# google/ffn

Hardware: AMD Instinct MI355X
Metric: FoV-steps/sec (flood-filling inference loop, 250^3 volume) (higher is better)
Workload: dtype f32 (fp16 hi + scaled-residual split products on the fp16 MFMA, f32 accumulate)

## Files before the change

ffn_amd/_lib.py:

```python

from __future__ import annotations

import ctypes
import os
import subprocess
import threading

_HERE = os.path.dirname(os.path.abspath(__file__))
CSRC = os.path.join(_HERE, 'csrc')
LIB_PATH = os.environ.get('FFN_AMD_LIB') or os.path.join(CSRC, 'libffn_hip.so')
HEADER = os.path.join(os.path.dirname(_HERE), 'include', 'ffn_hip.h')
HEADERS = [HEADER,
           os.path.join(os.path.dirname(_HERE), 'include', 'ffn_hip_debug.h'),
           os.path.join(os.path.dirname(_HERE), 'include', 'ffn_labels.h'),
           os.path.join(os.path.dirname(_HERE), 'include', 'ffn_seeds.h'),
           os.path.join(os.path.dirname(_HERE), 'include', 'ffn_decision.h'),
           os.path.join(os.path.dirname(_HERE), 'include', 'ffn_analysis.h'),
           os.path.join(os.path.dirname(_HERE), 'include', 'ffn_partitions.h'),
           os.path.join(os.path.dirname(_HERE), 'include', 'ffn_coordinates.h'),
           os.path.join(os.path.dirname(_HERE), 'include', 'ffn_evaluation.h'),
           os.path.join(os.path.dirname(_HERE), 'include', 'ffn_gradients.h'),
           os.path.join(os.path.dirname(_HERE), 'include', 'ffn_optimizer.h')]
SOURCES = ['ffn_hip.hip', 'ffn_canvas.hip', 'ffn_options.hip', 'ffn_labels.hip',
           'ffn_seeds.hip', 'ffn_decision.hip', 'ffn_analysis.hip',
# ... 81 lines not shown
              ('seed_got_too_weak', ctypes.c_int32),
              ('budget_exhausted', ctypes.c_int32),
              ('active', ctypes.c_int32),
              ('start_logit_known', ctypes.c_int32),
              ('start_logit', ctypes.c_float),
              ('min_pos', ctypes.c_int32 * 3),
              ('max_pos', ctypes.c_int32 * 3)]


class CommitCounts(ctypes.Structure):
  _fields_ = [('raw_segmented_voxels', ctypes.c_int64),
              ('actual_segmented_voxels', ctypes.c_int64),
              ('num_overlapped_ids', ctypes.c_int32)]


class TurnRequest(ctypes.Structure):
  _fields_ = [('do_commit', ctypes.c_int32),
              ('lo', ctypes.c_int32 * 3), ('hi', ctypes.c_int32 * 3),
              ('segment_threshold', ctypes.c_float),
              ('min_segment_size', ctypes.c_int64),
              ('segment_id', ctypes.c_int32),
              ('max_existing_id', ctypes.c_int32),
              ('mark_mode', ctypes.c_int32),
              ('mark_pos', ctypes.c_int32 * 3),
              ('num_candidates', ctypes.c_int32),
              ('min_boundary_dist', ctypes.c_int32 * 3),
              ('do_init', ctypes.c_int32),
              ('init_value', ctypes.c_float)]


class TurnResult(ctypes.Structure):
  _fields_ = [('counts', CommitCounts), ('committed', ctypes.c_int32),
              ('chosen', ctypes.c_int32)]


class PairDesc(ctypes.Structure):
  _fields_ = [('probs', ctypes.c_void_p), ('seg', ctypes.c_void_p),
              ('id_a', ctypes.c_uint64), ('id_b', ctypes.c_uint64),
              ('box_zyx', ctypes.c_int32 * 3), ('off_zyx', ctypes.c_int32 * 3),
              ('shape_zyx', ctypes.c_int32 * 3), ('reserved', ctypes.c_int32)]


class EvaluationSectionPlan(ctypes.Structure):
  _fields_ = [('margin_yx', ctypes.c_int32 * 2), ('kind', ctypes.c_int32),
              ('z0', ctypes.c_int32), ('dy', ctypes.c_int32),
              ('dx', ctypes.c_int32), ('blank_value', ctypes.c_float),
              ('blur_sigma', ctypes.c_float)]


class EvaluationSection(ctypes.Structure):
  _fields_ = [('blank_mask', ctypes.c_uint8), ('blur_mask', ctypes.c_uint8),
              ('gray', ctypes.c_uint8), ('reserved', ctypes.c_uint8),
              ('blank_yx', ctypes.c_int32 * 2), ('blur_yx', ctypes.c_int32 * 2),
              ('contrast', ctypes.c_float), ('brightness', ctypes.c_float),
              ('gamma', ctypes.c_float)]


class EvaluationGeometry(ctypes.Structure):
  _fields_ = [('input_seed_zyx', ctypes.c_int32 * 3),
              ('input_image_zyx', ctypes.c_int32 * 3),
              ('pred_mask_zyx', ctypes.c_int32 * 3),
              ('deltas_zyx', ctypes.c_int32 * 3),
              ('canvas_zyx', ctypes.c_int32 * 3),
              ('image_patch_zyx', ctypes.c_int32 * 3),
              ('label_patch_zyx', ctypes.c_int32 * 3),
              ('eval_zyx', ctypes.c_int32 * 3),
# ... 20 lines not shown
    'ffn_engine_set_weights': (_I, [_P, _P, ctypes.c_size_t]),
    'ffn_engine_set_pred_size': (_I, [_P, _I3]),
    'ffn_engine_set_option': (_I, [_P, ctypes.c_char_p, _I]),
    'ffn_engine_get_option': (_I, [_P, ctypes.c_char_p,
                                   ctypes.POINTER(ctypes.c_int)]),
    'ffn_engine_set_profiling': (_I, [_P, _I]),
    'ffn_engine_get_profile': (_I, [_P, ctypes.POINTER(ctypes.c_double),
                                    ctypes.POINTER(ctypes.c_int64), _I]),
    'ffn_engine_get_profile_samples': (_I, [_P, _P, _I, _P]),
    'ffn_engine_synchronize': (_I, [_P]),
    'ffn_engine_debug_clocks': (_I, [_P, _P]),
    'ffn_engine_debug_workgroups': (_I, [_P, _P, _I]),
    'ffn_engine_debug_flow_trace': (_I, [_P, _P, _I]),
    'ffn_predict': (_I, [_P, _I, _P, _P, _P]),
    'ffn_predict_device': (_I, [_P, _I, _P, _P, _P]),
    'ffn_forward_resident': (_I, [_P, _I, _I]),
    'ffn_canvas_create': (_I, [_P, _P, _I3, ctypes.POINTER(_P)]),
    'ffn_canvas_create_u8': (_I, [_P, _P, _I3, ctypes.c_float, ctypes.c_float,
                                  ctypes.POINTER(_P)]),
    'ffn_canvas_destroy': (None, [_P]),
    'ffn_canvas_init_seed': (_I, [_P, _I3, ctypes.c_float]),
    'ffn_canvas_step': (_I, [_P, _I, ctypes.POINTER(_P),
                             ctypes.POINTER(StepRequest),
                             ctypes.POINTER(StepParams),
                             ctypes.POINTER(StepResult)]),
    'ffn_canvas_step_submit': (_I, [_P, _I, ctypes.POINTER(_P),
                                    ctypes.POINTER(StepRequest),
                                    ctypes.POINTER(StepParams),
                                    ctypes.POINTER(ctypes.c_uint32)]),
    'ffn_canvas_step_wait': (_I, [_P, ctypes.c_uint32,
                                  ctypes.POINTER(StepResult)]),
    'ffn_canvas_segment_at': (_I, [_P, _I3, ctypes.POINTER(SegmentParams), _I,
                                   ctypes.POINTER(SegmentResult)]),
    'ffn_canvas_segment_many': (_I, [_P, _I, _P, _P, _P, _P, _P, _P]),
    'ffn_canvas_segment_many_carry': (_I, [_P, _I, _P, _P, _P, _P, _P, _P,
                                           ctypes.c_int32]),
    'ffn_canvas_segment_history': (_I, [_P, ctypes.c_size_t, ctypes.c_size_t,
                                        _P, _P,
                                        ctypes.POINTER(ctypes.c_size_t)]),
    'ffn_canvas_read_points': (_I, [_P, _I, _P, _P, _P]),
    'ffn_canvas_write_seg_points': (_I, [_P, _I, _P, _P]),
    'ffn_canvas_any_segmented': (_I, [_P, _I3, _I3,
                                      ctypes.POINTER(ctypes.c_int32)]),
    'ffn_canvas_commit_count': (_I, [_P, _I3, _I3, ctypes.c_float,
                                     ctypes.c_int32,
                                     ctypes.POINTER(CommitCounts),
                                     ctypes.c_int32, _P, _P]),
    'ffn_canvas_commit_assign': (_I, [_P, _I3, _I3, ctypes.c_float,
                                      ctypes.c_int32]),
    'ffn_canvas_segment_turn': (_I, [_P, _P, _P, _P, ctypes.c_int32, _P, _P, _P, _P,
                                     _P]),
    'ffn_canvas_set_restrictor': (_I, [_P, _P, _P, _P, _I3, _I3, _I3,
                                       ctypes.c_int32]),
    'ffn_canvas_read_restriction': (_I, [_P, _I3, _I3, _P]),
    'ffn_canvas_take_restricted_skips': (_I, [_P,
                                              ctypes.POINTER(ctypes.c_int64)]),
    'ffn_canvas_read_seed': (_I, [_P, _I3, _I3, _P]),
    'ffn_canvas_read_segmentation': (_I, [_P, _I3, _I3, _P]),
    'ffn_canvas_write_seed': (_I, [_P, _I3, _I3, _P]),
    'ffn_canvas_write_segmentation': (_I, [_P, _I3, _I3, _P]),
    'ffn_labels_create': (_I, [_I, ctypes.POINTER(_P)]),
    'ffn_labels_destroy': (None, [_P]),
    'ffn_labels_pair_counts': (_I, [_P, _P, _P, _I, ctypes.c_size_t,
                                    ctypes.c_size_t, _P, _P, _P, _P,
                                    ctypes.POINTER(ctypes.c_size_t)]),
    'ffn_labels_apply_pair_labels': (_I, [_P, ctypes.c_size_t, _P, _P, _P]),
# ... 238 lines not shown
```

ffn_amd/csrc/ffn_engine.h:

```cpp
#ifndef FFN_ENGINE_H_
#define FFN_ENGINE_H_

#include <hip/hip_runtime.h>

#include <algorithm>
#include <chrono>
#include <cstdarg>
#include <cstdio>
#include <mutex>
#include <vector>

#include "ffn_internal.h"
#include "ffn_types.h"
#include "ffn_stack_plan.h"
#include "ffn_host_loop.h"

using namespace ffn;

__attribute__((format(printf, 2, 3))) inline int fail(int code, const char* fmt, ...) {
  char buf[512];
  va_list ap;
  va_start(ap, fmt);
  vsnprintf(buf, sizeof(buf), fmt, ap);
  va_end(ap);
// ... 143 lines not shown
  unsigned long long* h_turn_dev = nullptr;
  size_t turn_ncap = 0, turn_hcap = 0, turn_ocap = 0;
  bool turn_hist_clean = false;
  unsigned turn_seq = 0;

  int prof_mode = 0;
  std::vector<hipEvent_t> events;
  int events_used = 0;
  hipEvent_t ahead_ev[2] = {nullptr, nullptr};
  bool ahead_ev_pending = false;
  double conv_ms = 0.0;
  int64_t conv_launches = 0;
  std::vector<ffn_canvas*> canvases;
  int prof_every = 1;
  long stack_calls = 0;
  bool prof_now = false;
  int ablate = 0;
  std::vector<int> chain_launches_pending;
  std::vector<float> prof_samples;
};

struct ffn_canvas {
  ffn_engine* engine = nullptr;
  float* image = nullptr;
  uint8_t* image_u8 = nullptr;
  float* image_lut = nullptr;
  float* seed = nullptr;
  int32_t* seg = nullptr;
  int cz = 0, cy = 0, cx = 0;
  size_t nvox = 0;
  int dirty_lo[3] = {0, 0, 0};
  int dirty_hi[3] = {0, 0, 0};
  ffn_host::SegmentState loop;
  hipEvent_t ev_util = nullptr;
  bool util_pending = false;
  bool paste_after_flag = false;
  int hint_n = 0;
  int hint_pos[kSpecMax][3] = {};
  bool hint_from_loop = false;
  unsigned long long* restrict_planes = nullptr;
  size_t restrict_plane_words = 0;
  int restrict_row_words = 0;
  std::vector<uint64_t> restrict_host;

  void mark_dirty(const int lo[3], const int hi[3]) {
    const int dims[3] = {cz, cy, cx};
    const bool empty = dirty_lo[0] >= dirty_hi[0];
    for (int k = 0; k < 3; ++k) {
      const int l = std::max(lo[k], 0), h = std::min(hi[k], dims[k]);
      dirty_lo[k] = empty ? l : std::min(dirty_lo[k], l);
      dirty_hi[k] = empty ? h : std::max(dirty_hi[k], h);
    }
  }
};

inline long long steady_ns() {
  return std::chrono::duration_cast<std::chrono::nanoseconds>(
             std::chrono::steady_clock::now().time_since_epoch()).count();
}
inline unsigned next_tag(unsigned t) { return t + 1 ? t + 1 : 1; }
inline void drop_spec(ffn_engine* e) {
  if (e->spec.valid && !e->ahead_valid) e->range_tag = next_tag(e->range_tag);
  if (e->ahead_valid) e->stat_ahead_wasted += 1;
  e->spec.valid = false;
  e->ahead_valid = false;
}
// ... 132 lines not shown
```

ffn_amd/csrc/ffn_hip.hip:

```cpp

#include <hip/hip_runtime.h>
#include <hip/hip_ext.h>

#include <algorithm>
#include <cmath>
#include <cstdarg>
#include <cstdio>
#include <cstdlib>
#include <cstring>
#include <map>
#include <mutex>
#include <string>
#include <vector>

#include "ffn_engine.h"
#include "ffn_kernels.h"
#include "ffn_step_kernels.h"
#include "ffn_conv_exact.h"
#include "ffn_conv_split.h"
#include "ffn_conv_resident.h"
#include "ffn_conv_half.h"

namespace {
thread_local std::string g_error;
// ... 1640 lines not shown
    drop_spec(e);
  }
  rc = ffn_canvas_step_submit(e, n, canvases, requests, params, &ticket);
  if (rc) return rc;
  return step_wait_impl(e, ticket, results, nullptr);
}

namespace {
int check_segment_params(const ffn_canvas* c, const ffn_segment_params& p, int resume, int k) {
  if (p.prefetch < 0 || p.prefetch > FFN_MAX_CANDIDATES)
    return fail(FFN_ERR_ARG, "prefetch must be 0..%d", FFN_MAX_CANDIDATES);
  if (p.shape_zyx[0] != c->cz || p.shape_zyx[1] != c->cy || p.shape_zyx[2] != c->cx)
    return k < 0 ? fail(FFN_ERR_ARG, "shape_zyx does not match the canvas")
                 : fail(FFN_ERR_ARG, "shape_zyx does not match canvas %d", k);
  for (int a = 0; a < 3; ++a)
    if (p.deltas_zyx[a] < 0 || p.margin_zyx[a] < 0)
      return fail(FFN_ERR_ARG, "negative deltas / margin");
  if (resume && !c->loop.active)
    return k < 0 ? fail(FFN_ERR_STATE, "no segment to resume")
                 : fail(FFN_ERR_STATE, "canvas %d: no segment to resume", k);
  return FFN_OK;
}

struct HipLoopDevice {
  ffn_canvas* c;
  int step(const ffn_step_request& req, const ffn_step_params& params,
           ffn_step_result* res) {
    ffn_canvas* one = c;
    return ffn_canvas_step(c->engine, 1, &one, &req, &params, res);
  }
  int read_point(const int32_t pos[3], float* seed, int32_t* seg) {
    return ffn_canvas_read_points(c, 1, pos, seed, seg);
  }
  void hint_next(int n, const int32_t (*pos)[3]) {
    EngineLock lock_(c->engine);
    c->hint_from_loop = true;
    c->hint_n = n < kSpecMax ? n : kSpecMax;
    for (int j = 0; j < c->hint_n; ++j)
      for (int a = 0; a < 3; ++a) c->hint_pos[j][a] = pos[j][a];
  }
};
}

namespace {
int resolve_many_carry_locked(ffn_engine* e) {
  if (!e->many_carry.active) return FFN_OK;
  HipLoopDevice dev{e->many_canvases.empty() ? nullptr : e->many_canvases[0]};
  auto wait = [&](ffn_step_result* res) {
    return step_wait_impl(e, e->many_ticket, res, nullptr);
  };
  const int rc = ffn_host::resolve_carry(&e->many_carry, dev, wait);
  e->many_canvases.clear();
  return rc;
}
}

}

int resolve_many_carry(ffn_engine* e, const ffn_canvas* only) {
  std::lock_guard<std::mutex> guard(e->many_mu);
  if (only && std::find(e->many_canvases.begin(), e->many_canvases.end(), only) ==
                  e->many_canvases.end())
    return FFN_OK;
  return resolve_many_carry_locked(e);
}

extern "C" {

int ffn_canvas_segment_at(ffn_canvas* c, const int32_t start[3],
                          const ffn_segment_params* p, int resume,
                          ffn_segment_result* out) {
  if (!c || !start || !p || !out) return fail(FFN_ERR_ARG, "null argument");
  if (!c->engine) return fail(FFN_ERR_STATE, "canvas outlived its engine");
  if (int rc = resolve_many_carry(c->engine, c)) return rc;
  if (int rc = check_segment_params(c, *p, resume, -1)) return rc;
  HipLoopDevice dev{c};
  ffn_host::SegmentLoop<HipLoopDevice> loop(dev, c->loop, *p);
  return loop.run(start, resume, out);
}

int ffn_canvas_segment_many(ffn_engine* e, int n, ffn_canvas* const* canvases,
                            const int32_t (*starts)[3],
                            const ffn_segment_params* params, const int32_t* resume,
                            ffn_segment_result* results, int32_t* finished) {
  return ffn_canvas_segment_many_carry(e, n, canvases, starts, params, resume, results,
                                       finished, 0);
}

int ffn_canvas_segment_many_carry(ffn_engine* e, int n, ffn_canvas* const* canvases,
                                  const int32_t (*starts)[3],
                                  const ffn_segment_params* params,
                                  const int32_t* resume, ffn_segment_result* results,
                                  int32_t* finished, int32_t carry) {
  if (!e || !canvases || !starts || !params || !resume || !results || !finished)
    return fail(FFN_ERR_ARG, "null argument");
  if (n < 1 || n > e->max_batch)
    return fail(FFN_ERR_ARG, "batch %d outside [1, %d]", n, e->max_batch);
  std::vector<HipLoopDevice> devs(n);
  std::vector<ffn_host::SegmentState*> states(n);
  for (int k = 0; k < n; ++k) {
    ffn_canvas* c = canvases[k];
    if (!c) return fail(FFN_ERR_ARG, "null canvas");
    if (c->engine != e) return fail(FFN_ERR_ARG, "canvas %d is not of this engine", k);
    for (int k2 = 0; k2 < k; ++k2)
      if (canvases[k2] == c) return fail(FFN_ERR_ARG, "canvas appears twice");
    const ffn_segment_params& p = params[k];
    if (int rc = check_segment_params(c, p, resume[k], k)) return rc;
    if (std::memcmp(&p.step, &params[0].step, sizeof(ffn_step_params)) != 0)
      return fail(FFN_ERR_ARG, "canvas %d: step parameters differ from canvas 0's", k);
    devs[k].c = c;
    states[k] = &c->loop;
// ... 38 lines not shown
```

ffn_amd/csrc/ffn_host_loop.h:

```cpp
#pragma once

#include <cstdlib>
#include <algorithm>
#include <cstdint>
#include <cstring>
#include <deque>
#include <unordered_map>
#include <unordered_set>
#include <vector>

#include "../../include/ffn_hip.h"

namespace ffn_host {

struct Coord {
  int32_t z, y, x;
  bool operator==(const Coord& o) const { return z == o.z && y == o.y && x == o.x; }
};

struct CoordHash {
  size_t operator()(const Coord& c) const {
    uint64_t h = (uint64_t)(uint32_t)c.z * 0x9E3779B97F4A7C15ull;
    h ^= (uint64_t)(uint32_t)c.y * 0xC2B2AE3D27D4EB4Full + (h << 6) + (h >> 2);
    h ^= (uint64_t)(uint32_t)c.x * 0x165667B19E3779F9ull + (h << 6) + (h >> 2);
    return (size_t)h;
  }
};

inline int32_t floordiv(int32_t a, int32_t b) {
  int32_t q = a / b;
  if ((a % b != 0) && (a < 0)) --q;
  return q;
}

struct SegmentState {
  struct Entry {
// ... 352 lines not shown
        m.rel[axis] = off;
        m.rel[o0] = fi - d_[o0];
        m.rel[o1] = fj - d_[o1];
        m.seg = res.face_seg[k];
        moves[nm++] = m;
      }
    }
    std::sort(moves, moves + nm, [](const Move& a, const Move& b) {
      if (a.score != b.score) return a.score > b.score;
      for (int i = 0; i < 3; ++i)
        if (a.rel[i] != b.rel[i]) return a.rel[i] > b.rel[i];
      return a.seg > b.seg;
    });
    for (int i = 0; i < nm; ++i) {
      if (i > 0 && moves[i].score == moves[i - 1].score &&
          moves[i].rel[0] == moves[i - 1].rel[0] &&
          moves[i].rel[1] == moves[i - 1].rel[1] &&
          moves[i].rel[2] == moves[i - 1].rel[2])
        continue;
      const Coord c{moves[i].rel[0] + pos.z, moves[i].rel[1] + pos.y,
                    moves[i].rel[2] + pos.x};
      push(moves[i].score, c);
      st_.cache.emplace(c, std::make_pair(moves[i].score, moves[i].seg));
    }
  }

  Dev& dev_;
  SegmentState& st_;
  const ffn_segment_params& p_;
  int32_t d_[3], dh_[3], dm_[3];
  int64_t steps_ = 0;
};

template <class Dev, class Wait>
int resolve_carry(ManyCarry* carry, Dev& any_dev, Wait&& wait) {
  if (!carry || !carry->active) return FFN_OK;
  std::vector<ffn_step_result> res(carry->items.size());
  const int rc = wait(res.data());
  carry->active = false;
  if (rc == FFN_OK) {
    for (size_t b = 0; b < carry->items.size(); ++b) {
      ManyCarry::Item& it = carry->items[b];
      SegmentLoop<Dev> loop(any_dev, *it.st, it.params);
      loop.consume(it.pd, res[b]);
      it.st->many_steps += 1;
    }
  }
  carry->items.clear();
  return rc;
}

template <class Dev, class BatchStep, class Submit, class Wait>
int segment_many(int n, Dev* devs, SegmentState* const* states,
                 const int32_t (*starts)[3], const ffn_segment_params* params,
                 const int32_t* resume, ffn_segment_result* out, int32_t* finished,
                 BatchStep&& batch_step, ManyCarry* carry, Submit&& submit,
                 Wait&& wait) {
  typedef SegmentLoop<Dev> Loop;
  for (int k = 1; k < n; ++k)
    if (std::memcmp(&params[k].step, &params[0].step, sizeof(ffn_step_params)) != 0)
      return FFN_ERR_ARG;
  const int rc_carry = resolve_carry(carry, devs[0], wait);
  std::vector<Loop> loops;
  loops.reserve(n);
  std::vector<char> running(n, 1);
  std::vector<typename Loop::Pending> pend(n);
// ... 76 lines not shown
```

ffn_amd/engine.py:

```python

from __future__ import annotations

import atexit
import ctypes
import threading
from typing import Sequence
import weakref

import numpy as np

from . import _lib
from ._lib import (CommitCounts, StepParams, StepRequest, StepResult, check, i3)


def _f32(a):
  return np.ascontiguousarray(a, dtype=np.float32)


_LIVE_ENGINES = weakref.WeakSet()


@atexit.register
def _close_all_engines():
  for eng in list(_LIVE_ENGINES):
# ... 16 lines not shown


def segment_many_with_retry(once, n, sarr, parr, rarr, before, fallback):
  res = (_lib.SegmentResult * n)()
  fin = (ctypes.c_int32 * n)()
  keys = list(range(n))
  sa, pa, ra, cur_res, cur_fin = sarr, parr, rarr, res, fin
  for attempt in range(MAX_VOID_REPEATS + 1):
    rc = once(keys, sa, pa, ra, cur_res, cur_fin)
    if cur_res is not res:
      for j, k in enumerate(keys):
        ctypes.pointer(res[k])[0] = cur_res[j]
        fin[k] = cur_fin[j]
    if rc not in _lib.ERR_VOIDED or attempt == MAX_VOID_REPEATS:
      return rc, res, fin
    fallback(rc)
    keys = [k for k in keys if not fin[k]]
    if not keys:
      return 0, res, fin
    m = len(keys)
    sa = (ctypes.c_int32 * 3 * m)()
    pa = (_lib.SegmentParams * m)()
    ra = (ctypes.c_int32 * m)(*([1] * m))
    cur_res = (_lib.SegmentResult * m)()
    cur_fin = (ctypes.c_int32 * m)()
    for j, k in enumerate(keys):
      for a in range(3):
        sa[j][a] = sarr[k][a]
      ctypes.pointer(pa[j])[0] = parr[k]
      if parr[k].max_steps > 0:
        spent = int(res[k].num_steps) - before[k]
        pa[j].max_steps = max(parr[k].max_steps - spent, 1)
  return rc, res, fin


class HipEngine:

  def __init__(self, fov_zyx, deltas_zyx, depth: int, features: int = 32,
               max_batch: int = 1, device_id: int = 0):
    self._lib = _lib.load()
    self._h = ctypes.c_void_p()
    self.fov_zyx = tuple(int(v) for v in fov_zyx)
    self.deltas_zyx = tuple(int(v) for v in deltas_zyx)
    self.depth = int(depth)
    self.features = int(features)
    self.max_batch = int(max_batch)
    self.device_id = int(device_id)
    check(self._lib.ffn_engine_create(self.device_id, i3(self.fov_zyx),
                                      i3(self.deltas_zyx), self.depth,
                                      self.features, self.max_batch,
                                      ctypes.byref(self._h)))
    self._canvas_arr = (ctypes.c_void_p * self.max_batch)()
    self._req_arr = (StepRequest * self.max_batch)()
    self._res_arr = (StepResult * self.max_batch)()
    self._slot_canvas_arr = [(ctypes.c_void_p * self.max_batch)()
                             for _ in range(2)]
    self._slot_req_arr = [(StepRequest * self.max_batch)() for _ in range(2)]
    self._slot_res_arr = [(StepResult * self.max_batch)() for _ in range(2)]
    self._submit_slot = 0
    self._ticket_slot = {}
    self._step_lock = threading.RLock()
    self.range_fallbacks = 0
    self.flow_fallbacks = 0
    self.variant_is_explicit = False
    self._default_variant = self.get_option('conv_variant')
    self.pred_zyx = self.fov_zyx
# ... 267 lines not shown
  def init_seed(self, pos, value: float):
    check(self._lib.ffn_canvas_init_seed(self._h, i3(pos), float(value)))

  def read_point(self, pos):
    self._pt[0], self._pt[1], self._pt[2] = int(pos[0]), int(pos[1]), int(pos[2])
    check(self._lib.ffn_canvas_read_points(
        self._h, 1, ctypes.addressof(self._pt), ctypes.addressof(self._pt_seed),
        ctypes.addressof(self._pt_seg)))
    return self._pt_seed.value, self._pt_seg.value

  def segment_at(self, start_pos, params: '_lib.SegmentParams',
                 resume: bool = False) -> '_lib.SegmentResult':
    res = _lib.SegmentResult()
    rc = self._lib.ffn_canvas_segment_at(self._h, i3(start_pos),
                                         ctypes.byref(params), int(resume),
                                         ctypes.byref(res))
    budget = params.max_steps
    summed = ('num_steps', 'skip_threshold', 'skip_invalid_pos', 'gate_rejects')
    before = dict.fromkeys(summed, 0)
    for _ in range(MAX_VOID_REPEATS):
      if rc not in _lib.ERR_VOIDED:
        break
      self.engine.voided(rc)
      for name in summed:
        before[name] += getattr(res, name)
      if budget > 0:
        params.max_steps = max(budget - before['num_steps'], 1)
      rc = self._lib.ffn_canvas_segment_at(self._h, i3(start_pos),
                                           ctypes.byref(params), 1,
                                           ctypes.byref(res))
    params.max_steps = budget
    for name in summed:
      setattr(res, name, getattr(res, name) + before[name])
    check(rc)
    return res

  def segment_history(self):
    total = ctypes.c_size_t(0)
    check(self._lib.ffn_canvas_segment_history(self._h, 0, 0, None, None,
                                               ctypes.byref(total)))
    n = total.value
    pos = np.empty((n, 3), np.int32)
    deleted = np.empty(n, np.uint32)
    if n:
      check(self._lib.ffn_canvas_segment_history(
          self._h, 0, n, pos.ctypes.data, deleted.ctypes.data, None))
    return pos, deleted

  def read_points(self, pos: np.ndarray):
    pos = np.ascontiguousarray(pos, dtype=np.int32).reshape(-1, 3)
    seed = np.empty(len(pos), np.float32)
    seg = np.empty(len(pos), np.int32)
    if len(pos):
      check(self._lib.ffn_canvas_read_points(self._h, len(pos), pos.ctypes.data,
                                             seed.ctypes.data, seg.ctypes.data))
    return seed, seg

  def write_seg_points(self, pos: np.ndarray, values: np.ndarray):
    pos = np.ascontiguousarray(pos, dtype=np.int32).reshape(-1, 3)
    values = np.ascontiguousarray(values, dtype=np.int32).ravel()
    assert len(pos) == len(values)
    if len(pos):
      check(self._lib.ffn_canvas_write_seg_points(
          self._h, len(pos), pos.ctypes.data, values.ctypes.data))

  def any_segmented(self, lo, hi) -> bool:
# ... 124 lines not shown
```

ffn_amd/inference/inference.py:

```python

from __future__ import annotations

import collections
import inspect
import ctypes

import logging
import os
import struct
import sys
import threading
import weakref
import time

import numpy as np
from scipy.special import expit
from scipy.special import logit

from .. import _lib
from .. import engine as hip_engine
from ..training import model as ffn_model
from . import executor
from . import movement
from . import seed as seed_lib
# ... 676 lines not shown
    else:
      image = np.ascontiguousarray(self.image, dtype=np.float32)
    self._handle = self._exec_client.create_canvas(image)
    self.seed = _DeviceArray(self, 'seed')
    self.segmentation = _DeviceArray(self, 'seg')
    if self.keep_probability_maps:
      self.seg_prob = storage.NumpyArray(shape=self.shape, dtype=np.uint8)
    else:
      self.seg_prob = None

  def _call(self, fn, *args, **kwargs):
    return self._exec_client.canvas_call(fn, *args, **kwargs)

  def close(self):
    if self._handle is not None:
      self._call(self._handle.close)
      self._handle = None

  def __del__(self):
    try:
      self.close()
    except Exception:
      pass
    super().__del__()

  def _invalidate_cache(self):
    self._cache = {}
    self._cached_start = None
    self._turn_rec = None

  TURN_CANDIDATES = int(os.environ.get('FFN_AMD_TURN_CANDIDATES', '128'))

  def _turn_ok(self) -> bool:
    ok = self.__dict__.get('_turn_static')
    if ok is None:
      ok = (hasattr(self._handle, 'segment_turn') and
            not self.keep_probability_maps and self._restrictor_ok())
      self._turn_static = ok
    return (ok and not self._checkpoint_due() and self.TURN_CANDIDATES > 0 and
            getattr(self.is_valid_pos, '__func__', None)
            is DeviceCanvas.is_valid_pos)

  def _policy_list(self):
    policy = self.__dict__.get('seed_policy')
    if getattr(type(policy), '__next__', None) is not seed_lib.BaseSeedPolicy.__next__:
      return None, None
    return getattr(policy, 'coords', None), getattr(policy, 'idx', None)

  def _is_current_seed(self, pos) -> bool:
    coords, idx = self._policy_list()
    return (coords is not None and idx is not None and
            1 <= idx <= len(coords) and
            tuple(int(v) for v in coords[idx - 1]) == pos)

  def _upcoming_seeds(self, first=None):
    coords, idx = self._policy_list()
    if coords is None or idx is None:
      return [] if first is None else [first]
    if first is not None:
      if not (1 <= idx <= len(coords) and
              tuple(int(v) for v in coords[idx - 1]) == first):
        return [first]
      idx -= 1
    out, listed = [], set()
    for c in np.asarray(coords[idx:idx + self.TURN_CANDIDATES]).tolist():
      c = (int(c[0]), int(c[1]), int(c[2]))
      if not self._in_bounds(c) or c in listed:
        break
      listed.add(c)
      out.append(c)
    return out

# ... 137 lines not shown
    t_done = time.time()
    self.t_last_predict = t_done
    hot[2] += t_done - t_call
    pred = self._finish_step(res)
    hot[0] += 1
    hot[1] += time.time() - t_start
    return pred

  def update_at(self, pos):
    return self._drive(self._update_at_gen(pos))

  def segment_at(self, start_pos, dynamic_image=None, vis_update_every=10,
                 vis_fixed_z=False, partial_segment_iters=0):
    del dynamic_image, vis_update_every, vis_fixed_z
    return self._drive(self._segment_at_gen(start_pos, partial_segment_iters))

  NATIVE_LOOP = os.environ.get('FFN_AMD_NATIVE_LOOP', '1') != '0'

  def _native_loop_ok(self) -> bool:
    ok = self.__dict__.get('_native_ok')
    if ok is None:
      cls = type(self)
      ok = (cls.NATIVE_LOOP and
            hasattr(self._handle, 'segment_at') and
            getattr(self._exec_client, 'in_thread', False) and
            type(self.movement_policy) is movement.FaceMaxMovementPolicy and
            self._restrictor_ok() and
            cls._segment_at_gen is DeviceCanvas._segment_at_gen)
      self._native_ok = ok
    return (ok and
            getattr(self.update_at, '__func__', None) is DeviceCanvas.update_at
            and getattr(self.is_valid_pos, '__func__', None)
            is DeviceCanvas.is_valid_pos)

  def _segment_params(self):
    sp = self.__dict__.get('_seg_params')
    if sp is None:
      sp = _lib.SegmentParams()
      policy = self.movement_policy
      sp.score_threshold = float(policy.score_threshold)
      for a in range(3):
        sp.deltas_zyx[a] = int(policy.deltas[a])
        sp.margin_zyx[a] = int(self._margin_t[a])
        sp.shape_zyx[a] = int(self.shape[a])
      sp.prefetch = self.PREFETCH
      sp.keep_history = 1 if self._keep_history else 0
      self._seg_params = sp
    sp.step = self._step_params
    return sp

  def _native_prelude(self, start_pos, resume=False):
    sp = self._segment_params()
    if not resume:
      if self.reset_seed_per_segment:
        self.init_seed(start_pos)
      self.reset_state(start_pos, reset_extents=self.reset_seed_per_segment)
      if self.movement_policy or self._min_pos is None:
        return None
      for a in range(3):
        sp.init_min_pos[a] = int(self._min_pos[a])
        sp.init_max_pos[a] = int(self._max_pos[a])
      cs = self._cached_start
      sp.initial_start_logit = (cs[1] if cs is not None and cs[0] == start_pos
                                else float('nan'))
    return sp

# ... 189 lines not shown
      while sid in self.origins:
        sid += 1
      out = self._turn(([int(v) for v in sel_lo], [int(v) for v in sel_hi], thr,
                        int(self.options.min_segment_size), sid, max_existing),
                       (pos, 2))
      raw, actual, ids, counts, committed = out[:5]
      if not committed:
        return raw, actual, ids, counts, None
      got = self.get_next_segment_id()
      assert got == sid, (got, sid)
      return raw, actual, ids, counts, sid
    raw, actual, ids, counts = self._call(self._handle.commit_count, sel_lo,
                                          sel_hi, thr, max_existing)
    if actual < self.options.min_segment_size:
      return raw, actual, ids, counts, None
    sid = self.get_next_segment_id()
    if self.keep_probability_maps:
      sel = tuple(slice(l, h) for l, h in zip(sel_lo, sel_hi))
      seed = self._call(self._handle.read_seed, sel_lo, sel_hi)
      seg = self._call(self._handle.read_segmentation, sel_lo, sel_hi)
      mask = (seed >= thr) & (seg <= 0)
      self.seg_prob[sel][mask] = storage.quantize_probability(
          expit(seed[mask]))
    self._invalidate_cache()
    self._call(self._handle.commit_assign, sel_lo, sel_hi, thr, sid)
    return raw, actual, ids, counts, sid

  def _set_segmentation(self, seg):
    self.segmentation[...] = np.asarray(seg, np.int32)

  def _set_seed(self, seed):
    self.seed[...] = np.asarray(seed, np.float32)
    self._turn_armed = False


class NativeSegment:

  __slots__ = ('start_pos', 'params', 'started')

  def __init__(self, start_pos, params):
    self.start_pos = start_pos
    self.params = params
    self.started = False


class MultiCanvasDriver:

  def __init__(self, engine, batch_size=None, overlap=True,
               max_steps_per_canvas=None, native=None, groups=1, carry=None):
    self.engine = engine
    hip_engine.pin_batched_arithmetic(engine)
    self.batch_size = batch_size or engine.max_batch
    self.overlap = overlap
    if native is None:
      native = os.environ.get('FFN_AMD_NATIVE_MANY', '1') != '0'
    self.native = bool(native) and hasattr(engine, 'segment_many')
    self.groups = max(1, int(groups)) if self.native else 1
    if carry is None:
      carry = os.environ.get('FFN_AMD_MANY_CARRY', '1') != '0'
    self.carry = bool(carry)
    self.max_steps_per_canvas = max_steps_per_canvas
    self.calls = 0
    self.steps = 0
    self.library_seconds = 0.0
    self.segments_ended = 0

# ... 249 lines not shown
```

ffn_amd/inference/seed.py:

```python

from __future__ import annotations

import itertools
import logging
import threading
import weakref

import numpy as np
from scipy import ndimage


class BaseSeedPolicy:

  def __init__(self, canvas, **kwargs):
    del kwargs
    self.canvas = weakref.proxy(canvas)
    self.coords = None
    self.idx = 0

  def init_coords(self):
    raise NotImplementedError()

  def __iter__(self):
    return self

  def __next__(self):
    if self.coords is None:
      self.init_coords()
      if self.coords is None:
        raise StopIteration()
      if self.coords.size:
        margin = np.array(self.canvas.margin)[np.newaxis, ...]
        self.coords = self.coords[np.all(
            (self.coords - margin >= 0) &
            (self.coords + margin < self.canvas.shape), axis=1), :]
    while self.idx < self.coords.shape[0]:
      curr = self.coords[self.idx, :]
      self.idx += 1
      return tuple(int(v) for v in curr)
    raise StopIteration()

  def next(self):
    return self.__next__()

  def get_state(self, previous=False):
    if previous:
      return self.coords, max(0, self.idx - 1)
    return self.coords, self.idx

  def set_state(self, state):
    self.coords, self.idx = state

  def get_exclusion_mask(self):
    mask = np.asarray(self.canvas.segmentation) > 0
    if self.canvas.restrictor is not None:
      if self.canvas.restrictor.mask is not None:
        mask |= self.canvas.restrictor.mask
      if self.canvas.restrictor.seed_mask is not None:
        mask |= self.canvas.restrictor.seed_mask
    return mask


def _ensure_spacing(coords, spacing, p_norm):
  if len(coords) < 2 or spacing <= 0:
    return coords
  from scipy.spatial import cKDTree
  near = cKDTree(coords).query_ball_point(coords, r=spacing, p=p_norm)
  rejected = set()
# ... 331 lines not shown
```

include/ffn_hip.h:

```cpp
#ifndef FFN_HIP_H_
#define FFN_HIP_H_

#include <stddef.h>
#include <stdint.h>

#ifdef __cplusplus
extern "C" {
#endif

#define FFN_OK 0
#define FFN_ERR_ARG (-1)
#define FFN_ERR_HIP (-2)
#define FFN_ERR_STATE (-3)
#define FFN_ERR_RANGE (-4)

#define FFN_ERR_FLOW (-5)

#define FFN_MAX_CANDIDATES 16

typedef struct ffn_engine ffn_engine;
typedef struct ffn_canvas ffn_canvas;

typedef struct ffn_step_params {
  float pad_value;
// ... 126 lines not shown
                            int64_t* overlap_counts);
int ffn_canvas_commit_assign(ffn_canvas* canvas, const int32_t lo[3],
                             const int32_t hi[3], float segment_threshold,
                             int32_t segment_id);

typedef struct ffn_turn_request {
  int32_t do_commit;
  int32_t lo[3], hi[3];
  float   segment_threshold;
  int64_t min_segment_size;
  int32_t segment_id;
  int32_t max_existing_id;
  int32_t mark_mode;
  int32_t mark_pos[3];
  int32_t num_candidates;
  int32_t min_boundary_dist[3];
  int32_t do_init;
  float   init_value;
} ffn_turn_request;

typedef struct ffn_turn_result {
  ffn_commit_counts counts;
  int32_t committed;
  int32_t chosen;
} ffn_turn_result;

int ffn_canvas_segment_turn(ffn_canvas* canvas, const ffn_turn_request* request,
                            const int32_t* candidates ,
                            ffn_turn_result* result, int32_t max_overlaps,
                            int32_t* overlap_ids, int64_t* overlap_counts,
                            int32_t* cand_flags, float* cand_seed,
                            int32_t* cand_seg);

int ffn_canvas_set_restrictor(ffn_canvas* canvas, const uint8_t* mask,
                              const uint8_t* seed_mask, const uint8_t* shift_mask,
                              const int32_t shift_shape[3], const int32_t pre[3],
                              const int32_t post[3], int32_t scale);
int ffn_canvas_read_restriction(ffn_canvas* canvas, const int32_t lo[3],
                                const int32_t hi[3], uint8_t* dst);
int ffn_canvas_take_restricted_skips(ffn_canvas* canvas, int64_t* count);

int ffn_canvas_read_seed(ffn_canvas* canvas, const int32_t lo[3],
                         const int32_t hi[3], float* dst);
int ffn_canvas_read_segmentation(ffn_canvas* canvas, const int32_t lo[3],
                                 const int32_t hi[3], int32_t* dst);
int ffn_canvas_write_seed(ffn_canvas* canvas, const int32_t lo[3],
                          const int32_t hi[3], const float* src);
int ffn_canvas_write_segmentation(ffn_canvas* canvas, const int32_t lo[3],
                                  const int32_t hi[3], const int32_t* src);

int ffn_engine_set_profiling(ffn_engine* engine, int mode);
int ffn_engine_get_profile(ffn_engine* engine, double* conv_ms_total,
                           int64_t* conv_launches, int reset);
int ffn_engine_get_profile_samples(ffn_engine* engine, float* out_ms, int max_n, int* n);
int ffn_engine_set_pred_size(ffn_engine* engine, const int32_t pred_zyx[3]);
int ffn_engine_set_option(ffn_engine* engine, const char* name, int value);
int ffn_engine_get_option(ffn_engine* engine, const char* name, int* value);
int ffn_engine_synchronize(ffn_engine* engine);

const char* ffn_last_error(void);
int ffn_abi_version(void);

#ifdef __cplusplus
}
#endif
#endif
// ... 1 lines not shown
```

Before: 5346.

## Move the per-seed segmentation loop into a native batched seed-loop call

Adds ffn_canvas_segment_all, a C++ SeedLoop that walks the seed list, filters candidates through segment turns, runs each segment, and records commit or reject outcomes for up to a budget of segments per call. The Python inference loop hands whole batches of seeds to this call and replays the per-seed records into counters and overlaps afterwards. The aim is to remove the Python overhead and ctypes round-trips that come with each seed. In exchange it adds a large amount of state-handling code (resume after voided errors, overlap buffer offsets, budgets and deadlines) that must match the existing Python semantics.

```diff
diff --git a/ffn_amd/_lib.py b/ffn_amd/_lib.py
--- a/ffn_amd/_lib.py
+++ b/ffn_amd/_lib.py
@@ -137,6 +137,49 @@
 class TurnResult(ctypes.Structure):
   _fields_ = [('counts', CommitCounts), ('committed', ctypes.c_int32),
               ('chosen', ctypes.c_int32)]
+
+
+SEED_NO_STEPS, SEED_WEAK, SEED_TOO_SMALL, SEED_COMMITTED = 0, 1, 2, 3
+
+
+class SeedRecord(ctypes.Structure):
+  _fields_ = [('pos', ctypes.c_int32 * 3), ('outcome', ctypes.c_int32),
+              ('segment_id', ctypes.c_int32), ('num_overlaps', ctypes.c_int32),
+              ('first_overlap', ctypes.c_int64),
+              ('raw_segmented_voxels', ctypes.c_int64),
+              ('actual_segmented_voxels', ctypes.c_int64),
+              ('seconds', ctypes.c_double), ('segment', SegmentResult)]
+
+
+class SeedLoopArgs(ctypes.Structure):
+  _fields_ = [('seeds', ctypes.c_void_p), ('num_seeds', ctypes.c_int64),
+              ('first_seed', ctypes.c_int64), ('segment', SegmentParams),
+              ('min_boundary_dist', ctypes.c_int32 * 3),
+              ('init_value', ctypes.c_float),
+              ('segment_threshold', ctypes.c_float),
+              ('half_pred', ctypes.c_int32 * 3),
+              ('min_segment_size', ctypes.c_int64),
+              ('next_segment_id', ctypes.c_int32),
+              ('max_existing_id', ctypes.c_int32),
+              ('turn_candidates', ctypes.c_int32), ('resume', ctypes.c_int32),
+              ('max_segments', ctypes.c_int32), ('has_deadline', ctypes.c_int32),
+              ('max_ms', ctypes.c_double), ('deadline_s', ctypes.c_double),
+              ('max_records', ctypes.c_int32), ('reserved', ctypes.c_int32),
+              ('records', ctypes.c_void_p), ('max_overlaps', ctypes.c_int64),
+              ('overlap_ids', ctypes.c_void_p),
+              ('overlap_counts', ctypes.c_void_p)]
+
+
+class SeedLoopResult(ctypes.Structure):
+  _fields_ = [('next_seed', ctypes.c_int64), ('num_overlaps', ctypes.c_int64),
+              ('rejected_invalid', ctypes.c_int64),
+              ('rejected_segmented', ctypes.c_int64),
+              ('rejected_restricted', ctypes.c_int64),
+              ('rejected_too_close', ctypes.c_int64),
+              ('restricted_skips', ctypes.c_int64),
+              ('seconds', ctypes.c_double), ('num_records', ctypes.c_int32),
+              ('turns', ctypes.c_int32), ('exhausted', ctypes.c_int32),
+              ('in_segment', ctypes.c_int32)]
 
 
 class PairDesc(ctypes.Structure):
@@ -223,6 +266,8 @@
                                   ctypes.POINTER(StepResult)]),
     'ffn_canvas_segment_at': (_I, [_P, _I3, ctypes.POINTER(SegmentParams), _I,
                                    ctypes.POINTER(SegmentResult)]),
+    'ffn_canvas_segment_all': (_I, [_P, ctypes.POINTER(SeedLoopArgs),
+                                    ctypes.POINTER(SeedLoopResult)]),
     'ffn_canvas_segment_many': (_I, [_P, _I, _P, _P, _P, _P, _P, _P]),
     'ffn_canvas_segment_many_carry': (_I, [_P, _I, _P, _P, _P, _P, _P, _P,
                                            ctypes.c_int32]),
diff --git a/ffn_amd/csrc/ffn_engine.h b/ffn_amd/csrc/ffn_engine.h
--- a/ffn_amd/csrc/ffn_engine.h
+++ b/ffn_amd/csrc/ffn_engine.h
@@ -199,6 +199,7 @@
   int dirty_lo[3] = {0, 0, 0};
   int dirty_hi[3] = {0, 0, 0};
   ffn_host::SegmentState loop;
+  ffn_host::SeedLoopState seed_loop;
   hipEvent_t ev_util = nullptr;
   bool util_pending = false;
   bool paste_after_flag = false;
diff --git a/ffn_amd/csrc/ffn_hip.hip b/ffn_amd/csrc/ffn_hip.hip
--- a/ffn_amd/csrc/ffn_hip.hip
+++ b/ffn_amd/csrc/ffn_hip.hip
@@ -1696,6 +1696,12 @@
   int read_point(const int32_t pos[3], float* seed, int32_t* seg) {
     return ffn_canvas_read_points(c, 1, pos, seed, seg);
   }
+  int turn(const ffn_turn_request& rq, const int32_t* cand, ffn_turn_result* out,
+           int32_t max_overlaps, int32_t* ids, int64_t* counts, int32_t* flags,
+           float* cand_seed, int32_t* cand_seg) {
+    return ffn_canvas_segment_turn(c, &rq, cand, out, max_overlaps, ids, counts, flags,
+                                   cand_seed, cand_seg);
+  }
   void hint_next(int n, const int32_t (*pos)[3]) {
     EngineLock lock_(c->engine);
     c->hint_from_loop = true;
@@ -1741,6 +1747,21 @@
   HipLoopDevice dev{c};
   ffn_host::SegmentLoop<HipLoopDevice> loop(dev, c->loop, *p);
   return loop.run(start, resume, out);
+}
+
+int ffn_canvas_segment_all(ffn_canvas* c, const ffn_seed_loop_args* a,
+                           ffn_seed_loop_result* out) {
+  if (!c || !a || !out) return fail(FFN_ERR_ARG, "null argument");
+  if (!c->engine) return fail(FFN_ERR_STATE, "canvas outlived its engine");
+  if (!ffn_host::seed_loop_args_ok(*a))
+    return fail(FFN_ERR_ARG, "seed list, candidates, records or overlap arrays");
+  if (int rc = resolve_many_carry(c->engine, c)) return rc;
+  if (int rc = check_segment_params(c, a->segment, 0, -1)) return rc;
+  if (a->resume && !(c->seed_loop.in_segment && c->loop.active))
+    return fail(FFN_ERR_STATE, "no segment to resume");
+  HipLoopDevice dev{c};
+  ffn_host::SeedLoop<HipLoopDevice> loop(dev, c->loop, c->seed_loop, *a, out);
+  return loop.run();
 }
 
 int ffn_canvas_segment_many(ffn_engine* e, int n, ffn_canvas* const* canvases,
diff --git a/ffn_amd/csrc/ffn_host_loop.h b/ffn_amd/csrc/ffn_host_loop.h
--- a/ffn_amd/csrc/ffn_host_loop.h
+++ b/ffn_amd/csrc/ffn_host_loop.h
@@ -2,6 +2,8 @@
 
 #include <cstdlib>
 #include <algorithm>
+#include <chrono>
+#include <climits>
 #include <cstdint>
 #include <cstring>
 #include <deque>
@@ -420,6 +422,208 @@
   int64_t steps_ = 0;
 };
 
+struct SeedLoopState {
+  bool in_segment = false;
+  ffn_seed_record rec{};
+};
+
+template <class Dev>
+class SeedLoop {
+ public:
+  SeedLoop(Dev& dev, SegmentState& st, SeedLoopState& sl, const ffn_seed_loop_args& a,
+           ffn_seed_loop_result* out)
+      : dev_(dev), st_(st), sl_(sl), a_(a), out_(out) {}
+
+  int run() {
+    std::memset(out_, 0, sizeof(*out_));
+    t0_ = Clock::now();
+    idx_ = a_.first_seed;
+    next_id_ = a_.next_segment_id;
+    max_id_ = a_.max_existing_id;
+    const int cap = a_.turn_candidates;
+    std::vector<int32_t> win(3 * (size_t)cap), flags(cap), cseg(cap);
+    std::vector<float> cseed(cap);
+    ffn_turn_request rq;
+    std::memset(&rq, 0, sizeof(rq));
+    for (int k = 0; k < 3; ++k) rq.min_boundary_dist[k] = a_.min_boundary_dist[k];
+    rq.do_init = 1;
+    rq.init_value = a_.init_value;
+    bool owed = false;
+    int rc = FFN_OK;
+    if (a_.resume) {
+      if (!sl_.in_segment) return FFN_ERR_STATE;
+      rc = segment(nullptr, &rq, &owed);
+    } else {
+      sl_.in_segment = false;
+    }
+    while (rc == FFN_OK) {
+      const bool go_on = attempts_ == 0 || !budget_spent();
+      const int n = go_on ? window(win.data(), cap) : 0;
+      if (!owed && n == 0) {
+        if (!go_on) break;
+        if (idx_ >= a_.num_seeds) {
+          out_->exhausted = 1;
+          break;
+        }
+        ++out_->rejected_invalid;
+        ++idx_;
+        continue;
+      }
+      rq.num_candidates = n;
+      ffn_turn_result tr;
+      const int64_t room = a_.max_overlaps - out_->num_overlaps;
+      rc = dev_.turn(rq, win.data(), &tr, (int32_t)std::min<int64_t>(room, INT32_MAX),
+                     a_.overlap_ids + out_->num_overlaps,
+                     a_.overlap_counts + out_->num_overlaps, flags.data(), cseed.data(),
+                     cseg.data());
+      if (rc) break;
+      ++out_->turns;
+      if (owed) settle(tr, &rq);
+      owed = false;
+      if (!go_on) break;
+      int chosen = -1;
+      for (int k = 0; k < n && chosen < 0; ++k) {
+        if (flags[k] == 3) break;
+        ++idx_;
+        switch (flags[k]) {
+          case 0: chosen = k; break;
+          case 1: ++out_->rejected_invalid, ++out_->rejected_segmented; break;
+          case 2: ++out_->rejected_too_close; break;
+          default: ++out_->rejected_restricted; break;
+        }
+      }
+      if (chosen >= 0) rc = segment(&win[3 * (size_t)chosen], &rq, &owed);
+    }
+    out_->next_seed = idx_;
+    out_->in_segment = sl_.in_segment ? 1 : 0;
+    out_->restricted_skips = st_.skip_restricted;
+    st_.skip_restricted = 0;
+    out_->seconds = since(t0_);
+    return rc;
+  }
+
+ private:
+  typedef std::chrono::steady_clock Clock;
+  static double since(Clock::time_point t) {
+    return std::chrono::duration<double>(Clock::now() - t).count();
+  }
+
+  bool budget_spent() const {
+    const double s = since(t0_);
+    return (a_.max_segments > 0 && attempts_ >= a_.max_segments) ||
+           (a_.max_ms > 0 && s * 1e3 >= a_.max_ms) ||
+           (a_.has_deadline && s >= a_.deadline_s) ||
+           out_->num_records >= a_.max_records ||
+           a_.max_overlaps - out_->num_overlaps < 2 * ((int64_t)max_id_ + 1);
+  }
+
+  bool in_bounds(const int32_t* p) const {
+    for (int k = 0; k < 3; ++k)
+      if (p[k] - a_.segment.margin_zyx[k] < 0 ||
+          p[k] + a_.segment.margin_zyx[k] >= a_.segment.shape_zyx[k])
+        return false;
+    return true;
+  }
+
+  int window(int32_t* win, int cap) {
+    listed_.clear();
+    int n = 0;
+    for (int64_t i = idx_; i < a_.num_seeds && n < cap; ++i, ++n) {
+      const int32_t* p = a_.seeds + 3 * i;
+      if (!in_bounds(p) || !listed_.insert(Coord{p[0], p[1], p[2]}).second) break;
+      std::memcpy(win + 3 * n, p, 12);
+    }
+    return n;
+  }
+
+  int segment(const int32_t* start, ffn_turn_request* rq, bool* owed) {
+    ffn_seed_record& rec = sl_.rec;
+    ffn_segment_params p = a_.segment;
+    p.max_steps = 0;
+    const int resume = start ? 0 : 1;
+    if (start) {
+      std::memset(&rec, 0, sizeof(rec));
+      for (int k = 0; k < 3; ++k)
+        rec.pos[k] = p.init_min_pos[k] = p.init_max_pos[k] = start[k];
+      p.initial_start_logit = a_.init_value;
+    }
+    const Clock::time_point t = Clock::now();
+    ffn_segment_result res;
+    SegmentLoop<Dev> loop(dev_, st_, p);
+    const int rc = loop.run(rec.pos, resume, &res);
+    rec.seconds += since(t);
+    res.num_steps += rec.segment.num_steps;
+    res.skip_threshold += rec.segment.skip_threshold;
+    res.skip_invalid_pos += rec.segment.skip_invalid_pos;
+    res.gate_rejects += rec.segment.gate_rejects;
+    rec.segment = res;
+    sl_.in_segment = rc != FFN_OK;
+    if (rc) return rc;
+    ++attempts_;
+    *owed = true;
+    if (res.num_steps <= 0) {
+      rec.outcome = FFN_SEED_NO_STEPS;
+      *owed = false;
+    } else if (res.start_logit_known && res.start_logit < p.step.move_threshold) {
+      rec.outcome = FFN_SEED_WEAK;
+      rq->mark_mode = 1;
+    } else {
+      rec.outcome = FFN_SEED_TOO_SMALL;
+      rq->do_commit = 1;
+      for (int k = 0; k < 3; ++k) {
+        rq->lo[k] = std::max(res.min_pos[k] - a_.half_pred[k], 0);
+        rq->hi[k] = std::min(res.max_pos[k] + a_.half_pred[k] + 1, p.shape_zyx[k]);
+      }
+      rq->segment_threshold = a_.segment_threshold;
+      rq->min_segment_size = a_.min_segment_size;
+      rq->segment_id = next_id_;
+      rq->max_existing_id = max_id_;
+      rq->mark_mode = 2;
+    }
+    for (int k = 0; k < 3; ++k) rq->mark_pos[k] = rec.pos[k];
+    a_.records[out_->num_records++] = rec;
+    return FFN_OK;
+  }
+
+  void settle(const ffn_turn_result& tr, ffn_turn_request* rq) {
+    ffn_seed_record& rec = a_.records[out_->num_records - 1];
+    if (rq->do_commit) {
+      rec.raw_segmented_voxels = tr.counts.raw_segmented_voxels;
+      rec.actual_segmented_voxels = tr.counts.actual_segmented_voxels;
+      rec.num_overlaps = tr.counts.num_overlapped_ids;
+      rec.first_overlap = out_->num_overlaps;
+      out_->num_overlaps += rec.num_overlaps;
+      if (tr.committed) {
+        rec.outcome = FFN_SEED_COMMITTED;
+        rec.segment_id = next_id_;
+        max_id_ = std::max(max_id_, next_id_);
+        ++next_id_;
+      }
+    }
+    rq->do_commit = 0;
+    rq->mark_mode = 0;
+  }
+
+  Dev& dev_;
+  SegmentState& st_;
+  SeedLoopState& sl_;
+  const ffn_seed_loop_args& a_;
+  ffn_seed_loop_result* out_;
+  Clock::time_point t0_;
+  int64_t idx_ = 0;
+  int32_t next_id_ = 0, max_id_ = 0, attempts_ = 0;
+  std::unordered_set<Coord, CoordHash> listed_;
+};
+
+inline bool seed_loop_args_ok(const ffn_seed_loop_args& a) {
+  return a.num_seeds >= 0 && (a.seeds || a.num_seeds == 0) && a.first_seed >= 0 &&
+         a.first_seed <= a.num_seeds && a.turn_candidates >= 1 &&
+         a.turn_candidates <= 4096 && a.max_records >= 1 && a.records &&
+         a.overlap_ids && a.overlap_counts && a.max_existing_id >= 0 &&
+         a.next_segment_id > 0 &&
+         a.max_overlaps >= 2 * ((int64_t)a.max_existing_id + 1);
+}
+
 template <class Dev, class Wait>
 int resolve_carry(ManyCarry* carry, Dev& any_dev, Wait&& wait) {
   if (!carry || !carry->active) return FFN_OK;
diff --git a/ffn_amd/engine.py b/ffn_amd/engine.py
--- a/ffn_amd/engine.py
+++ b/ffn_amd/engine.py
@@ -72,6 +72,44 @@
         spent = int(res[k].num_steps) - before[k]
         pa[j].max_steps = max(parr[k].max_steps - spent, 1)
   return rc, res, fin
+
+
+def seed_loop_with_retry(once, args, fallback):
+  total = _lib.SeedLoopResult()
+  saved = _lib.SeedLoopArgs.from_buffer_copy(args)
+  summed = ('rejected_invalid', 'rejected_segmented', 'rejected_restricted',
+            'rejected_too_close', 'restricted_skips', 'seconds', 'turns')
+  recs = ctypes.cast(args.records, ctypes.POINTER(_lib.SeedRecord))
+  try:
+    for attempt in range(MAX_VOID_REPEATS + 1):
+      res = _lib.SeedLoopResult()
+      rc = once(args, res)
+      n0, o0 = total.num_records, total.num_overlaps
+      for k in range(n0, n0 + res.num_records):
+        recs[k].first_overlap += o0
+        if recs[k].outcome == _lib.SEED_COMMITTED:
+          args.max_existing_id = max(args.max_existing_id, recs[k].segment_id)
+          args.next_segment_id = recs[k].segment_id + 1
+      for name in summed:
+        setattr(total, name, getattr(total, name) + getattr(res, name))
+      total.num_records = n0 + res.num_records
+      total.num_overlaps = o0 + res.num_overlaps
+      total.next_seed, total.exhausted = res.next_seed, res.exhausted
+      total.in_segment = res.in_segment
+      if rc not in _lib.ERR_VOIDED or attempt == MAX_VOID_REPEATS:
+        return rc, total
+      fallback(rc)
+      args.resume = 1
+      args.first_seed = res.next_seed
+      if saved.max_segments > 0:
+        args.max_segments = max(saved.max_segments - total.num_records, 1)
+      args.records = saved.records + total.num_records * ctypes.sizeof(_lib.SeedRecord)
+      args.max_records = saved.max_records - total.num_records
+      args.overlap_ids = saved.overlap_ids + 4 * total.num_overlaps
+      args.overlap_counts = saved.overlap_counts + 8 * total.num_overlaps
+      args.max_overlaps = saved.max_overlaps - total.num_overlaps
+  finally:
+    ctypes.pointer(args)[0] = saved
 
 
 class HipEngine:
@@ -405,6 +443,14 @@
     params.max_steps = budget
     for name in summed:
       setattr(res, name, getattr(res, name) + before[name])
+    check(rc)
+    return res
+
+  def segment_all(self, args: '_lib.SeedLoopArgs') -> '_lib.SeedLoopResult':
+    rc, res = seed_loop_with_retry(
+        lambda a, r: self._lib.ffn_canvas_segment_all(self._h, ctypes.byref(a),
+                                                      ctypes.byref(r)),
+        args, self.engine.voided)
     check(rc)
     return res
 
diff --git a/ffn_amd/inference/inference.py b/ffn_amd/inference/inference.py
--- a/ffn_amd/inference/inference.py
+++ b/ffn_amd/inference/inference.py
@@ -732,12 +732,19 @@
   TURN_CANDIDATES = int(os.environ.get('FFN_AMD_TURN_CANDIDATES', '128'))
 
   def _turn_ok(self) -> bool:
+    ok = self._turn_possible()
+    return ok and not self._checkpoint_due() and self._turn_unhooked()
+
+  def _turn_possible(self) -> bool:
     ok = self.__dict__.get('_turn_static')
     if ok is None:
       ok = (hasattr(self._handle, 'segment_turn') and
             not self.keep_probability_maps and self._restrictor_ok())
       self._turn_static = ok
-    return (ok and not self._checkpoint_due() and self.TURN_CANDIDATES > 0 and
+    return ok
+
+  def _turn_unhooked(self) -> bool:
+    return (self.TURN_CANDIDATES > 0 and
             getattr(self.is_valid_pos, '__func__', None)
             is DeviceCanvas.is_valid_pos)
 
@@ -941,6 +948,170 @@
             getattr(self.update_at, '__func__', None) is DeviceCanvas.update_at
             and getattr(self.is_valid_pos, '__func__', None)
             is DeviceCanvas.is_valid_pos)
+
+  NATIVE_SEED_LOOP = os.environ.get('FFN_AMD_NATIVE_SEED_LOOP', '1') != '0'
+  SEED_LOOP_SEGMENTS = int(os.environ.get('FFN_AMD_SEED_LOOP_SEGMENTS', '32'))
+  SEED_LOOP_MS = float(os.environ.get('FFN_AMD_SEED_LOOP_MS', '250'))
+
+  def _seed_loop_ok(self, policy) -> bool:
+    cls = type(self)
+    if not (self.NATIVE_SEED_LOOP and hasattr(self._handle, 'segment_all') and
+            self.reset_seed_per_segment and not self._keep_history):
+      return False
+    for name, stock in _SEED_LOOP_STOCK.items():
+      if name in self.__dict__ or getattr(cls, name, None) is not stock:
+        return False
+    if type(policy).__next__ is not seed_lib.BaseSeedPolicy.__next__:
+      return False
+    if self.origins and max(self.origins) > self._max_id:
+      return False
+    return (self._native_loop_ok() and self._turn_possible() and
+            self._turn_unhooked())
+
+  def segment_all(self, seed_policy=seed_lib.PolicyPeaks,
+                  partial_segment_iters=0):
+    if partial_segment_iters:
+      return super().segment_all(seed_policy, partial_segment_iters)
+    policy = seed_policy(self)
+    if not self._seed_loop_ok(policy):
+      return super().segment_all(lambda canvas: policy)
+    return self._segment_all_native(policy)
+
+  def _segment_all_native(self, policy):
+    self.seed_policy = policy
+    if self._seed_policy_state is not None:
+      policy.set_state(self._seed_policy_state)
+      self._seed_policy_state = None
+    c = self.counters
+    with timer_counter(c, 'segment_all'):
+      calls = c['seed-policy-calls']
+      c['seed-policy-time-ms']
+      if not policy.ensure_coords():
+        calls.Increment()
+      else:
+        args, recs = self._seed_loop_args(policy)
+        while True:
+          self._maybe_save_checkpoint(partial_segment_iters=0)
+          self._seed_loop_call_args(args, policy)
+          self._invalidate_cache()
+          res = self._call(self._handle.segment_all, args)
+          self.seed_loop_calls = self.__dict__.get('seed_loop_calls', 0) + 1
+          self._seed_loop_apply(args, res, recs, policy)
+          if res.exhausted:
+            calls.Increment()
+            break
+    self.log_info('Segmentation done.')
+    self._deregister_client()
+
+  def _seed_loop_args(self, policy):
+    args = _lib.SeedLoopArgs()
+    seeds = np.ascontiguousarray(policy.coords, dtype=np.int32).reshape(-1, 3)
+    args._seeds = seeds
+    args.seeds = seeds.ctypes.data
+    args.num_seeds = len(seeds)
+    ctypes.pointer(args.segment)[0] = self._segment_params()
+    args.segment.max_steps = 0
+    mbd = self.options.min_boundary_dist
+    args.min_boundary_dist[:] = [int(mbd.z), int(mbd.y), int(mbd.x)]
+    args.init_value = float(self.options.init_activation)
+    args.segment_threshold = float(self.options.segment_threshold)
+    args.half_pred[:] = [int(v) // 2 for v in self._pred_size]
+    args.min_segment_size = int(self.options.min_segment_size)
+    args.turn_candidates = self.TURN_CANDIDATES
+    args.max_segments = self.SEED_LOOP_SEGMENTS
+    args.max_ms = self.SEED_LOOP_MS
+    n = (self.SEED_LOOP_SEGMENTS if self.SEED_LOOP_SEGMENTS > 0 else 256) + 8
+    recs = (_lib.SeedRecord * n)()
+    args.records = ctypes.addressof(recs)
+    args.max_records = n
+    return args, recs
+
+  def _seed_loop_call_args(self, args, policy):
+    args.first_seed = int(policy.idx)
+    args.resume = 0
+    args.next_segment_id = self._max_id + 1
+    args.max_existing_id = self._max_id
+    need = 4 * (self._max_id + args.max_records + 2)
+    if args.max_overlaps < need:
+      args._ids = np.zeros(2 * need, np.int32)
+      args._counts = np.zeros(2 * need, np.int64)
+      args.overlap_ids = args._ids.ctypes.data
+      args.overlap_counts = args._counts.ctypes.data
+      args.max_overlaps = 2 * need
+    timed = self.checkpoint_path is not None and self.checkpoint_interval_sec > 0
+    args.has_deadline = 1 if timed else 0
+    args.deadline_s = (self.checkpoint_last + self.checkpoint_interval_sec -
+                       time.time()) if timed else 0.0
+
+  def _seed_loop_apply(self, args, res, recs, policy):
+    c = self.counters
+    consumed = int(res.next_seed) - int(policy.idx)
+    policy.idx = int(res.next_seed)
+    if consumed:
+      c['seed-policy-calls'].IncrementBy(consumed)
+    if res.rejected_invalid:
+      c['skip_invalid_pos'].IncrementBy(int(res.rejected_invalid))
+      self.gate_rejects += int(res.rejected_segmented)
+    if res.restricted_skips:
+      c['skip_restriced_pos'].IncrementBy(int(res.restricted_skips))
+    self.turns += int(res.turns)
+    self._turn_armed = True
+    last = None
+    for k in range(res.num_records):
+      rec = recs[k]
+      seg = rec.segment
+      pos = (int(rec.pos[0]), int(rec.pos[1]), int(rec.pos[2]))
+      n = int(seg.num_steps)
+      ms = rec.seconds * MSEC_IN_SEC
+      self.log_info('Starting segmentation at %r (zyx)', pos)
+      c['segment_at-loop-calls'].Increment()
+      c['segment_at-loop-time-ms'].IncrementBy(ms)
+      if n:
+        c['update_at-calls'].IncrementBy(n)
+        c['inference-calls'].IncrementBy(n)
+        c['predict-calls'].IncrementBy(n)
+        c['movement_policy-calls'].IncrementBy(n)
+        c['update_at-time-ms'].IncrementBy(ms)
+        c['inference-time-ms'].IncrementBy(ms)
+      if seg.skip_threshold:
+        c['skip_threshold'].IncrementBy(int(seg.skip_threshold))
+      if seg.skip_invalid_pos:
+        c['skip_invalid_pos'].IncrementBy(int(seg.skip_invalid_pos))
+      if seg.seed_got_too_weak:
+        c['seed_got_too_weak'].Increment()
+      self.gate_rejects += int(seg.gate_rejects)
+      last = (pos, seg)
+      if rec.outcome == _lib.SEED_NO_STEPS:
+        c['invalid-other-time-ms'].IncrementBy(ms)
+        self.log_info('Failed: num iters was %d', n)
+      elif rec.outcome == _lib.SEED_WEAK:
+        self.log_info('Failed: weak seed')
+        c['invalid-weak-time-ms'].IncrementBy(ms)
+      elif rec.outcome == _lib.SEED_TOO_SMALL:
+        self.log_info('Failed: too small: %d', int(rec.actual_segmented_voxels))
+        c['invalid-small-time-ms'].IncrementBy(ms)
+      else:
+        sid = int(rec.segment_id)
+        actual = int(rec.actual_segmented_voxels)
+        self._max_id = sid
+        c['voxels-segmented'].IncrementBy(actual)
+        c['voxels-overlapping'].IncrementBy(
+            int(rec.raw_segmented_voxels) - actual)
+        self.log_info('Created supervoxel:%d  seed(zyx):%s  size:%d  iters:%d',
+                      sid, pos, actual, n)
+        o = int(rec.first_overlap)
+        self.overlaps[sid] = np.array([args._ids[o:o + rec.num_overlaps],
+                                       args._counts[o:o + rec.num_overlaps]])
+        self.origins[sid] = storage.OriginInfo(pos, n, rec.seconds)
+        c['valid-time-ms'].IncrementBy(ms)
+    if last is not None:
+      pos, seg = last
+      self.reset_state(pos)
+      self._min_pos = np.array([int(v) for v in seg.min_pos])
+      self._max_pos = np.array([int(v) for v in seg.max_pos])
+      if seg.start_logit_known:
+        self._cached_start = (pos, float(seg.start_logit))
+      self.t_last_predict = time.time()
 
   def _segment_params(self):
     sp = self.__dict__.get('_seg_params')
@@ -1196,6 +1367,12 @@
   def _set_seed(self, seed):
     self.seed[...] = np.asarray(seed, np.float32)
     self._turn_armed = False
+
+
+_SEED_LOOP_STOCK = {
+    name: getattr(DeviceCanvas, name)
+    for name in ('_segment_at_native', '_segment_at_gen', '_segment_all_gen',
+                 '_commit', '_turn', 'init_seed', '_mark_excluded', '_too_close')}
 
 
 class NativeSegment:
diff --git a/ffn_amd/inference/seed.py b/ffn_amd/inference/seed.py
--- a/ffn_amd/inference/seed.py
+++ b/ffn_amd/inference/seed.py
@@ -24,16 +24,21 @@
   def __iter__(self):
     return self
 
-  def __next__(self):
+  def ensure_coords(self) -> bool:
     if self.coords is None:
       self.init_coords()
       if self.coords is None:
-        raise StopIteration()
+        return False
       if self.coords.size:
         margin = np.array(self.canvas.margin)[np.newaxis, ...]
         self.coords = self.coords[np.all(
             (self.coords - margin >= 0) &
             (self.coords + margin < self.canvas.shape), axis=1), :]
+    return True
+
+  def __next__(self):
+    if not self.ensure_coords():
+      raise StopIteration()
     while self.idx < self.coords.shape[0]:
       curr = self.coords[self.idx, :]
       self.idx += 1
diff --git a/include/ffn_hip.h b/include/ffn_hip.h
--- a/include/ffn_hip.h
+++ b/include/ffn_hip.h
@@ -182,6 +182,67 @@
                             int32_t* cand_flags, float* cand_seed,
                             int32_t* cand_seg);
 
+#define FFN_SEED_NO_STEPS  0
+#define FFN_SEED_WEAK      1
+#define FFN_SEED_TOO_SMALL 2
+#define FFN_SEED_COMMITTED 3
+
+typedef struct ffn_seed_record {
+  int32_t pos[3];
+  int32_t outcome;
+  int32_t segment_id;
+  int32_t num_overlaps;
+  int64_t first_overlap;
+  int64_t raw_segmented_voxels;
+  int64_t actual_segmented_voxels;
+  double  seconds;
+  ffn_segment_result segment;
+} ffn_seed_record;
+
+typedef struct ffn_seed_loop_args {
+  const int32_t* seeds;
+  int64_t num_seeds;
+  int64_t first_seed;
+  ffn_segment_params segment;
+  int32_t min_boundary_dist[3];
+  float   init_value;
+  float   segment_threshold;
+  int32_t half_pred[3];
+  int64_t min_segment_size;
+  int32_t next_segment_id;
+  int32_t max_existing_id;
+  int32_t turn_candidates;
+  int32_t resume;
+  int32_t max_segments;
+  int32_t has_deadline;
+  double  max_ms;
+  double  deadline_s;
+  int32_t max_records;
+  int32_t reserved;
+  ffn_seed_record* records;
+  int64_t max_overlaps;
+  int32_t* overlap_ids;
+  int64_t* overlap_counts;
+} ffn_seed_loop_args;
+
+typedef struct ffn_seed_loop_result {
+  int64_t next_seed;
+  int64_t num_overlaps;
+  int64_t rejected_invalid;
+  int64_t rejected_segmented;
+  int64_t rejected_restricted;
+  int64_t rejected_too_close;
+  int64_t restricted_skips;
+  double  seconds;
+  int32_t num_records;
+  int32_t turns;
+  int32_t exhausted;
+  int32_t in_segment;
+} ffn_seed_loop_result;
+
+int ffn_canvas_segment_all(ffn_canvas* canvas, const ffn_seed_loop_args* args,
+                           ffn_seed_loop_result* result);
+
 int ffn_canvas_set_restrictor(ffn_canvas* canvas, const uint8_t* mask,
                               const uint8_t* seed_mask, const uint8_t* shift_mask,
                               const int32_t shift_shape[3], const int32_t pre[3],
```

Result: faster. 5458 (median of 6 runs) (+2.1%).
